# MoonLab-YH/AOD_MEH_HUA

Measured on AMD Instinct MI355X. Metric: images/sec train+HUA-score, RetinaNet-R50 VOC 512^2, higher is better.
Workload: dtype bf16x3

## Files before the change

### aod_meh_hua_amd/_C.py

```python
import ctypes as C
import os

import torch

_HERE = os.path.dirname(os.path.abspath(__file__))
LIB_PATH = os.environ.get('AOD_HIP_LIB') or os.path.join(_HERE, 'lib', 'libaodhip.so')


class AodHipError(RuntimeError):
    pass


if not os.path.exists(LIB_PATH):
    raise ImportError(f'{LIB_PATH} is missing: run `python -m aod_meh_hua_amd.build` (hipcc, gfx950). '
                      'There is no CPU fallback for the MEH/HUA hot path.')
lib = C.CDLL(LIB_PATH)


class ConvSeg(C.Structure):
    _fields_ = [('B', C.c_int32), ('H', C.c_int32), ('W', C.c_int32), ('OH', C.c_int32), ('OW', C.c_int32),
                ('src_row0', C.c_int64), ('dst_row0', C.c_int64)]


class ConvDesc(C.Structure):
    _fields_ = [('C', C.c_int32), ('N', C.c_int32), ('R', C.c_int32), ('S', C.c_int32), ('stride', C.c_int32),
                ('pad', C.c_int32), ('dil', C.c_int32), ('transposed', C.c_int32), ('relu', C.c_int32),
                ('out_f32', C.c_int32), ('nseg', C.c_int32), ('x3', C.c_int32), ('seg', ConvSeg * 8)]


class ConvPlan(C.Structure):
    _fields_ = [(n, C.c_int32) for n in ('kind', 'bm', 'bn', 'nt', 'ops', 'stages', 'x3', 'grouped', 'ksplit', 'taps', 'wide', 'pre', 'lat', 'grid')]


P, I32, I64, F32, U64, SZ = C.c_void_p, C.c_int32, C.c_int64, C.c_float, C.c_uint64, C.c_size_t
_SIGS = {
    'aod_version': (C.c_int, []),
    'aod_conv_x3p_count': (C.c_int64, []),
    'aod_set_pointwise_mode': (C.c_int, [I32]),
    'aod_bottleneck64_fwd': (C.c_int, [P, I32, I32, I32, I32, P, P, P, P, P, P, P, P, P, P, P, P]),
    'aod_bottleneck64x3_fwd': (C.c_int, [P, I32, I32, I32, I32, P, P, P, P, P, P, P, P, P, P, P, P]),
    'aod_bottleneck64x3_ds_fwd': (C.c_int, [P, I32, I32, I32, P, P, P, P, P, P, P, P, P, P, P, P, P, P]),
    'aod_bottleneck64_ds_fwd': (C.c_int, [P, I32, I32, I32, P, P, P, P, P, P, P, P, P, P, P, P, P, P]),
    'aod_halo_conv3x3_x3_applies': (C.c_int, [P]),
    'aod_halo_conv3x3_x3': (C.c_int, [P, P, P, P, P, P]),
    'aod_mfma_clock_probe': (C.c_int, [I32, I32, P, P, P]),
    'aod_bottleneck128x3_bwd': (C.c_int, [P, I32, I32, I32, P, P, P, P, P, P, P, P, P, P, P, P, P]),
    'aod_bottleneck128x3_fwd': (C.c_int, [P, I32, I32, I32, P, P, P, P, P, P, P, P, P, P, P, P, P]),
    'aod_bottleneck128_fwd': (C.c_int, [P, I32, I32, I32, P, P, P, P, P, P, P, P, P, P, P, P, P]),
    'aod_frag_pack': (C.c_int, [P, I32, I32, P]),
    'aod_frag_pack_item_bytes': (C.c_int, []),
    'aod_bottleneck256f_fwd': (C.c_int, [P, I32, I32, I32, P, P, P, P, P, P, P, P, P, P, P, P, P]),
    'aod_bottleneck256f_bwd': (C.c_int, [P, I32, I32, I32, P, P, P, P, P, P, P, P, P, P, P, P, P]),
    'aod_bottleneck_bwd': (C.c_int, [I32, P, I32, I32, I32, P, P, P, P, P, P, P, P, P, P, P, P, P]),
    'aod_bottleneck256_fwd': (C.c_int, [P, I32, I32, I32, P, P, P, P, P, P, P, P, P, P, P, P, P]),
    'aod_conv2d': (C.c_int, [C.POINTER(ConvDesc), P, P, P, P, P, P, P, P, P, P, P]),
    'aod_conv2d_ws_bytes': (SZ, [C.POINTER(ConvDesc)]),
    'aod_conv2d_ws': (C.c_int, [C.POINTER(ConvDesc), P, P, P, P, P, P, P, P, P, P, P, SZ, P]),
    'aod_conv2d_plan': (C.c_int, [C.POINTER(ConvDesc), I32, C.c_uint, C.POINTER(ConvPlan)]),
    'aod_conv2d_grouped': (C.c_int, [C.POINTER(ConvDesc), I32, P, P, P, P, P, P, P]),
    'aod_halo_conv3x3_applies': (C.c_int, [C.POINTER(ConvDesc)]),
    'aod_halo_conv3x3': (C.c_int, [C.POINTER(ConvDesc), P, P, P, P, P, P, P]),
    'aod_conv2d_wgrad': (C.c_int, [C.POINTER(ConvDesc), P, P, P, P, P]),
    'aod_conv2d_wgrad_splits': (C.c_int, [C.POINTER(ConvDesc)]),
    'aod_conv2d_wgrad_slabs': (C.c_int, [C.POINTER(ConvDesc), P, P, P, I32, I64, P, P]),
    'aod_conv2d_wgrad_group_plan': (C.c_int, [P, I32, P]),
    'aod_conv2d_wgrad_grouped': (C.c_int, [P, I32, P, P, P, P, P, P, P]),
    'aod_unpack_wgrad_slabs_grouped': (C.c_int, [I32, P, P, P, P, P, P, P, P, P, P, P, P, P, P, P, P, P]),
    'aod_unpack_wgrad_slabs': (C.c_int, [P, I32, I64, P, I32, I32, I32, I32, I32, I32, P, P, P, P, P, P, P]),
    'aod_conv_row_table_bytes': (SZ, [C.POINTER(ConvDesc)]),
    'aod_conv_row_table': (C.c_int, [C.POINTER(ConvDesc), P, P]),
    'aod_pack_weight_fwd': (C.c_int, [P, P, I32, I32, I32, I32, I32, P]),
    'aod_param_prep': (C.c_int, [P, I32, I32, P]),
    'aod_param_prep_item_bytes': (C.c_int, []),
    'aod_pack_weight_dgrad': (C.c_int, [P, P, I32, I32, I32, I32, I32, P, P]),
    'aod_unpack_wgrad': (C.c_int, [P, P, I32, I32, I32, I32, I32, I32, I32, P, P, P, P, P, P, P]),
    'aod_nchw_f32_to_nhwc_bf16': (C.c_int, [P, P, I32, I32, I32, I32, I32, P]),
    'aod_nchw_f32_to_s2d_bf16': (C.c_int, [P, P, I32, I32, I32, I32, P]),
    'aod_stem_pool_fwd': (C.c_int, [P, P, P, P, P, I32, I32, I32, P]),
    'aod_set_deterministic': (C.c_int, [I32]),
    'aod_get_deterministic': (C.c_int, []),
    'aod_stem_pool_x3_fwd': (C.c_int, [P, P, P, P, P, I32, I32, I32, I32, P]),
    'aod_maxpool3x3s2': (C.c_int, [P, P, I32, I32, I32, I32, P]),
    'aod_upsample2x_add': (C.c_int, [P, P, I32, I32, I32, I32, I32, I32, P]),
    'aod_upsample2x_add_bwd': (C.c_int, [P, P, I32, I32, I32, I32, I32, I32, P]),
# ... 79 lines not shown
```

### aod_meh_hua_amd/csrc/conv.hip

```cpp
#include "common.h"
#include "pointwise.h"
#include "conv_x3p.h"

struct ConvGroup { const bf16_t* x; const bf16_t* w; void* y; const float* pre_shift; const bf16_t* mask; float* colsum; };
struct ConvKParams {
  const bf16_t* x;
  const bf16_t* w;
  void* y;
  const float* pre_scale;
  const float* pre_shift;
  const bf16_t* res;
  const bf16_t* mask;
  const float* post_scale;
  bf16_t* zraw;
  float* colsum;
  int C, N, K, R, S, stride, pad, dil, transposed, relu, out_f32;
  int nseg, M;
  int tiles_m, tiles_n;
  int ksplit;
  float* ws;
  int perm;
  int ngroups;
  ConvGroup grp[4];
  int stagger;
  int x3;
  int tap_inner;
  int bigrows;
  float* cs_ws;
  int up_w, up_hw;
  long long x_bytes, w_bytes;
  int segH[8], segW[8], segOH[8], segOW[8], segB[8];
  long long seg_src0[8], seg_dst0[8];
  int seg_mend[8];
};

#ifdef AOD_TILE_TIMING
__device__ unsigned long long* g_tile_stamps = nullptr;
extern "C" int aod_dbg_set_tile_stamps(void* buf) { return (int)hipMemcpyToSymbol(HIP_SYMBOL(g_tile_stamps), &buf, sizeof(buf)); }
#define TSTAMP(k) do { if (g_tile_stamps && threadIdx.x == 0) g_tile_stamps[(size_t)blockIdx.x * 16 + (k)] = wall_clock64(); } while (0)
#else
#define TSTAMP(k) do {} while (0)
#endif

__device__ __forceinline__ unsigned udiv_small(unsigned n, unsigned d) {
  unsigned q = (unsigned)((float)n * __builtin_amdgcn_rcpf((float)d));
  const int r = (int)(n - q * d);
  q = r < 0 ? q - 1 : ((unsigned)r >= d ? q + 1 : q);
  return q;
}

__device__ __forceinline__ int xcd_swizzle(int bid, int nwg) {
  const int q = nwg >> 3, r = nwg & 7, xcd = bid & 7, j = bid >> 3;
  return (xcd < r ? xcd * (q + 1) : r * (q + 1) + (xcd - r) * q) + j;
}

template <int BM, int BN, int NT, int OPS, bool GROUPED, int ST, bool X3>
__global__ __launch_bounds__(NT) __attribute__((amdgpu_waves_per_eu(BM >= 192 ? 2 : (NT == 512 ? 4 : 1), BM >= 192 ? 2 : (NT == 512 ? 4 : 8)))) void conv_igemm_kernel(const ConvKParams p) {
  static_assert(NT == 256 || NT == 512, "4 or 8 waves");
  static_assert(ST == 2 || (ST == 3 && NT == 256), "LDS stages: 2, or 3 for the 4-wave forms");
  static_assert(!X3 || NT == 256 || (NT == 512 && (BM == 256 || BM == 192 || BM == 128)), "X3: the 4-wave forms, the 8-wave 256 x 256 / 192 x 192 tiles and (A/B) the 8-wave 128 x 128 tile");
  constexpr int BK = 64;
  constexpr int CPR = BK / 8;
  constexpr int RPP = NT / CPR;
  constexpr int A_IT = BM / RPP, B_IT = BN / RPP;
  constexpr int ROWB = BK * 2;
  constexpr int A_BYTES = BM * ROWB, B_BYTES = BN * ROWB, STAGE = A_BYTES + B_BYTES;
  constexpr int WAVES_M = NT / 128;
  constexpr int WM = BM / WAVES_M, WN = BN / 2;
  constexpr int MI = WM / 16, NI = WN / 16;
  constexpr int CP = BN + 4;
  constexpr int EP = (BM * CP * 4 > 144 * 1024) ? 2 : 1;
  constexpr int EBM = BM / EP;
  constexpr bool PREFETCH = EP == 1 && !X3;
  extern __shared__ __attribute__((aligned(16))) char smem[];

  const int t = threadIdx.x;
  TSTAMP(0);
  const int lane = t & 63, wave = t >> 6;
  const int wm = wave >> 1, wn = wave & 1;
  const int nwg = p.tiles_m * p.tiles_n;
  int wg;
  if (!p.perm) wg = xcd_swizzle(blockIdx.x, nwg * (GROUPED ? p.ngroups : p.ksplit));
  else if ((nwg & 31) == 0) {
    const int x = blockIdx.x & 7, j = blockIdx.x >> 3, q = j & 3, k = j >> 2, tq = nwg >> 2;
    wg = q * tq + x * (tq >> 3) + k;
  } else wg = blockIdx.x;
  const int tile = wg % nwg, zz = wg / nwg;
  const int kz = GROUPED ? 0 : zz;
  const int gi = GROUPED ? zz : 0;
#define AOD_GSEL(f, dflt) (GROUPED ? (gi == 0 ? p.grp[0].f : (gi == 1 ? p.grp[1].f : (gi == 2 ? p.grp[2].f : p.grp[3].f))) : (dflt))
  const bf16_t* const g_x = AOD_GSEL(x, p.x);
  const bf16_t* const g_w = AOD_GSEL(w, p.w);
  const float* const g_shift = AOD_GSEL(pre_shift, p.pre_shift);
#define g_y AOD_GSEL(y, p.y)
#define g_mask AOD_GSEL(mask, p.mask)
#define g_colsum AOD_GSEL(colsum, p.colsum)
  const int tile_n = tile % p.tiles_n, tile_m = tile / p.tiles_n;
  const int m0 = tile_m * BM, n0 = tile_n * BN;
#ifdef AOD_TILE_TIMING
  if (m0 < 0) return;
  TSTAMP(8);
#endif

  const int uw = __builtin_amdgcn_readfirstlane(wave);
  const int prow = lane >> 3;
  const int kc = (lane & 7) ^ ((4 * uw + (lane >> 4)) & 7);
  const int C8 = p.C >> 3;
  const auto rsrc_x = __builtin_amdgcn_make_buffer_rsrc((void*)g_x, 0, (int)p.x_bytes, 0x00020000);
  const auto rsrc_w = __builtin_amdgcn_make_buffer_rsrc((void*)g_w, 0, (int)p.w_bytes, 0x00020000);
  constexpr unsigned OOB = 0xfffffff0u;

  unsigned rbase[A_IT];
  int ry0[A_IT], rx0[A_IT], rH[A_IT], rW[A_IT];
  auto seg_of = [&](int m) {
    int sg = 0;
    if (p.nseg > 1) {
#pragma unroll
      for (int q = 0; q < 7; ++q) sg += (m >= p.seg_mend[q]) ? 1 : 0;
    }
    return sg;
  };
  const int m_last = (m0 + BM < p.M ? m0 + BM : p.M) - 1;
  const int sg_first = seg_of(m0);
  const bool one_seg = sg_first == seg_of(m_last);
  struct Geo { unsigned mstart, OW, OH, ohw, B, H, W, src0b, imgb; };
  auto load_geo = [&](int sg) {
    Geo g;
    g.mstart = sg ? (unsigned)p.seg_mend[sg - 1] : 0u;
    g.OW = (unsigned)p.segOW[sg]; g.OH = (unsigned)p.segOH[sg]; g.ohw = g.OH * g.OW; g.B = (unsigned)p.segB[sg];
    g.H = (unsigned)p.segH[sg]; g.W = (unsigned)p.segW[sg];
    g.src0b = (unsigned)((unsigned long long)p.seg_src0[sg] * (unsigned)(p.C * 2));
    g.imgb = g.H * g.W * (unsigned)(p.C * 2);
    return g;
  };
  const Geo gu = load_geo(sg_first);
  auto udiv = [&](unsigned n, unsigned d) { return p.bigrows ? n / d : udiv_small(n, d); };
  auto rowpos = [&](unsigned ml, const Geo& g, unsigned& b, unsigned& oy, unsigned& ox, int& cls) {
    if (!p.perm) {
      b = udiv(ml, g.ohw);
      const unsigned rem = ml - b * g.ohw;
      oy = udiv(rem, g.OW); ox = rem - oy * g.OW; cls = 0;
    } else {
      const unsigned H0 = (g.OH + 1) >> 1, H1 = g.OH >> 1, W0 = (g.OW + 1) >> 1, W1 = g.OW >> 1;
      const unsigned e0 = g.B * H0 * W0, e1 = e0 + g.B * H0 * W1, e2 = e1 + g.B * H1 * W0;
      cls = (ml >= e0 ? 1 : 0) + (ml >= e1 ? 1 : 0) + (ml >= e2 ? 1 : 0);
      const unsigned start = cls == 0 ? 0u : (cls == 1 ? e0 : (cls == 2 ? e1 : e2));
      const unsigned Hc = (cls & 2) ? H1 : H0, Wc = (cls & 1) ? W1 : W0, hw = Hc * Wc;
      const unsigned r = ml - start;
      b = udiv(r, hw);
      const unsigned rem = r - b * hw, yy = udiv(rem, Wc);
      oy = 2 * yy + (unsigned)(cls >> 1); ox = 2 * (rem - yy * Wc) + (unsigned)(cls & 1);
// ... 563 lines not shown
#pragma unroll
        for (int j = 0; j < 8; ++j) zv[j] = (bf16_t)raw[j];
        *reinterpret_cast<bf16x8*>(p.zraw + off) = zv;
      }
    } else {
      for (int j = 0; j < 8 && n + j < p.N; ++j) {
        const long long off = drow * p.N + n + j;
        float u = v[j];
        if (p.pre_scale) u *= p.pre_scale[n + j];
        if (g_shift) u += g_shift[n + j];
        if (p.res) u += (float)p.res[off];
        if (g_mask) u = ((float)g_mask[off] > 0.f) ? u : 0.f;
        if (p.post_scale) u *= p.post_scale[n + j];
        if (p.relu) u = fmaxf(u, 0.f);
        csum[j] += u;
        if (p.out_f32) reinterpret_cast<float*>(g_y)[off] = u;
        else reinterpret_cast<bf16_t*>(g_y)[off] = (bf16_t)u;
        if (p.zraw) p.zraw[off] = (bf16_t)raw[j];
      }
    }
  }
  }
  TSTAMP(5);
#ifdef AOD_TILE_TIMING
  __builtin_amdgcn_s_waitcnt(0);
  asm volatile("s_waitcnt vmcnt(0)" ::: "memory");
  TSTAMP(6);
  if (g_tile_stamps && threadIdx.x == 0)
    g_tile_stamps[(size_t)blockIdx.x * 16 + 7] = ((unsigned long long)__builtin_amdgcn_s_getreg(63508) << 32) | (unsigned)__builtin_amdgcn_s_getreg(63492);
#endif
  if (g_colsum) {
    __syncthreads();
    float* sr = reinterpret_cast<float*>(smem);
#pragma unroll
    for (int j = 0; j < 8; ++j) if (ecok) sr[er * BN + ec * 8 + j] = csum[j];
    __syncthreads();
    if (t < BN && n0 + t < p.N) {
      float s = 0.f;
      for (int r = 0; r < NT / NCHT; ++r) s += sr[r * BN + t];
      if (p.cs_ws) p.cs_ws[((long long)gi * p.tiles_m + tile_m) * p.N + n0 + t] = s;
      else atomicAdd(g_colsum + n0 + t, s);
    }
  }
}

#undef g_y
#undef g_mask
#undef g_colsum
#undef AOD_GSEL

template <int BM, int BN, int NT = 256, int OPS = 2, bool GROUPED = false, int ST = 2, bool X3 = false>
static int launch_conv(const ConvKParams& p, hipStream_t st) {
  ConvKParams q = p;
  q.tiles_m = (p.M + BM - 1) / BM;
  q.tiles_n = (p.N + BN - 1) / BN;
  const size_t stage = (size_t)(BM + BN) * 128 * ST;
  const size_t epi_full = (size_t)BM * (BN + 4) * 4;
  const size_t epi = epi_full > 144 * 1024 ? epi_full / 2 : epi_full;
  const size_t lds = (stage > epi ? stage : epi) + (size_t)BM * 8;
  static unsigned long long attr_done = 0;
  if (aod_first_on_device(&attr_done)) {
    (void)hipFuncSetAttribute(reinterpret_cast<const void*>(&conv_igemm_kernel<BM, BN, NT, OPS, GROUPED, ST, X3>), hipFuncAttributeMaxDynamicSharedMemorySize, (int)lds);
  }
  bool any_cs = q.colsum != nullptr;
  if (GROUPED) for (int g = 0; g < q.ngroups; ++g) any_cs = any_cs || q.grp[g].colsum;
  const int ng = GROUPED ? q.ngroups : 1;
  if (q.ksplit == 1) q.cs_ws = any_cs ? aod_det_scratch((size_t)ng * q.tiles_m * q.N) : nullptr;
  hipLaunchKernelGGL((conv_igemm_kernel<BM, BN, NT, OPS, GROUPED, ST, X3>), dim3(q.tiles_m * q.tiles_n * (q.ngroups > 1 ? q.ngroups : q.ksplit)), dim3(NT), lds, st, q);
  if (q.ksplit == 1 && q.cs_ws) {
    for (int g = 0; g < ng; ++g) {
      float* dst = GROUPED ? q.grp[g].colsum : q.colsum;
      if (dst) { const int rc = aod_colsum_finalize(q.cs_ws + (size_t)g * q.tiles_m * q.N, q.tiles_m, q.N, q.N, dst, nullptr, 0, st); if (rc) return rc; }
    }
  }
  return 0;
}

static int fill_params(const aod_conv_desc_t* d, ConvKParams& p) {
  AOD_CHECK_ARG(d->nseg >= 1 && d->nseg <= 8, "conv: nseg %d out of range", d->nseg);
  AOD_CHECK_ARG(d->C % 8 == 0, "conv: source channels %d must be a multiple of 8", d->C);
  AOD_CHECK_ARG(d->stride >= 1 && d->dil >= 1 && d->R >= 1 && d->S >= 1, "conv: bad geometry");
  AOD_CHECK_ARG(d->x3 == 0 || d->x3 == 1, "conv: aod_conv_desc_t.x3 = %d (0 or 1; descriptors must be zero-initialised -- the field took the place of padding in aod_version() 2)", d->x3);
  p.C = d->C; p.N = d->N; p.R = d->R; p.S = d->S; p.K = d->R * d->S * d->C;
  p.stride = d->stride; p.pad = d->pad; p.dil = d->dil; p.transposed = d->transposed;
  p.relu = d->relu; p.out_f32 = d->out_f32; p.nseg = d->nseg; p.x3 = d->x3 ? 1 : 0;
  if (p.x3) AOD_CHECK_ARG(d->C % 64 == 0, "conv (x3): X-layout source width %d must be a multiple of 64", d->C);
  long long m = 0;
  for (int i = 0; i < d->nseg; ++i) {
    const aod_conv_seg_t& s = d->seg[i];
    if (!d->transposed) {
      const int eh = (s.H + 2 * d->pad - d->dil * (d->R - 1) - 1) / d->stride + 1;
      const int ew = (s.W + 2 * d->pad - d->dil * (d->S - 1) - 1) / d->stride + 1;
      AOD_CHECK_ARG(s.OH >= 1 && s.OW >= 1 && s.OH <= eh && s.OW <= ew, "conv: segment %d output %dx%d exceeds the expected %dx%d", i, s.OH, s.OW, eh, ew);
    } else {
      const int eh = (s.OH + 2 * d->pad - d->dil * (d->R - 1) - 1) / d->stride + 1;
      const int ew = (s.OW + 2 * d->pad - d->dil * (d->S - 1) - 1) / d->stride + 1;
      AOD_CHECK_ARG(eh == s.H && ew == s.W, "dgrad: segment %d dZ %dx%d != expected %dx%d", i, s.H, s.W, eh, ew);
    }
    AOD_CHECK_ARG(s.H < 65536 && s.W < 65536 && s.OH < 65536 && s.OW < 65536, "conv: segment %d image side >= 65536", i);
    p.segB[i] = s.B; p.segH[i] = s.H; p.segW[i] = s.W; p.segOH[i] = s.OH; p.segOW[i] = s.OW;
    p.seg_src0[i] = s.src_row0; p.seg_dst0[i] = s.dst_row0;
    m += (long long)s.B * s.OH * s.OW;
    AOD_CHECK_ARG(m < (1ll << 31), "conv: too many rows");
    p.seg_mend[i] = (int)m;
  }
  for (int i = d->nseg; i < 8; ++i) { p.segB[i] = p.segH[i] = p.segW[i] = p.segOH[i] = p.segOW[i] = 0; p.seg_src0[i] = p.seg_dst0[i] = 0; p.seg_mend[i] = (int)m; }
  p.M = (int)m;
  p.bigrows = 0;
// ... 59 lines not shown
        bf16x8 ov;
#pragma unroll
        for (int j = 0; j < 8; ++j) ov[j] = (bf16_t)v[j];
        *reinterpret_cast<bf16x8*>(reinterpret_cast<bf16_t*>(p.y) + off) = ov;
        if (xout) {
          bf16x8 ol;
#pragma unroll
          for (int j = 0; j < 8; ++j) ol[j] = (bf16_t)(v[j] - (float)ov[j]);
          *reinterpret_cast<bf16x8*>(reinterpret_cast<bf16_t*>(p.y) + off + 32) = ol;
        }
      } else {
        for (int j = 0; j < 8 && n + j < p.N; ++j) {
          if (p.out_f32) reinterpret_cast<float*>(p.y)[off + j] = v[j];
          else reinterpret_cast<bf16_t*>(p.y)[off + j] = (bf16_t)v[j];
        }
      }
      if (p.zraw)
        for (int j = 0; j < 8 && n + j < p.N; ++j) p.zraw[off + j] = (bf16_t)raw[j];
    }
  }
  if (p.colsum) {
#pragma unroll
    for (int j = 0; j < 8; ++j) sr[er][ec * 8 + j] = csum[j];
    __syncthreads();
    const int c = blockIdx.y * 256 + t;
    if (c < p.N) {
      float s2 = 0.f;
#pragma unroll
      for (int r = 0; r < 8; ++r) s2 += sr[r][t];
      if (p.cs_ws) p.cs_ws[(long long)blockIdx.x * p.N + c] = s2;
      else atomicAdd(p.colsum + c, s2);
    }
  }
}

struct ConvKnobs {
  struct Once {
    const char* ksplit_maxhw = getenv("AOD_KSPLIT_MAXHW");
    const char* ksplit_steps = getenv("AOD_KSPLIT_STEPS");
    const char* stagger = getenv("AOD_STAGGER");
    const char* x3_taps_inner = getenv("AOD_X3_TAPS_INNER");
    const char* dgrad_lattice = getenv("AOD_DGRAD_LATTICE");
    const char* dgrad_classes = getenv("AOD_DGRAD_CLASSES");
    const char* tile_want = getenv("AOD_TILE_WANT");
    const char* tile_256 = getenv("AOD_TILE_256");
    const char* x3_128_w8 = getenv("AOD_X3_128_W8");
    const char* x3_128_st3 = getenv("AOD_X3_128_ST3");
    const char* tile_w8 = getenv("AOD_TILE_W8");
    const char* ring3 = getenv("AOD_RING3");
  };
  static const Once& once() { static const Once k{}; return k; }

  enum Call { X3P_OVER_256, X3_TILE_192, X3P_GROUPED, X3P, X3P_PRE, X3P_BN, X3P_DGRAD, X3P_LATTICE, X3P_MIN_STEPS, X3P_PRE_MIN_STEPS, X3P_MIN_TILES,
              X3P_ROT, NCALL };
  const char* val[NCALL];
  unsigned seen = 0;
  const char* call(Call k) {
    static const char* const names[NCALL] = {"AOD_X3P_OVER_256", "AOD_X3_TILE_192", "AOD_X3P_GROUPED", "AOD_X3P", "AOD_X3P_PRE", "AOD_X3P_BN",
                                             "AOD_X3P_DGRAD", "AOD_X3P_LATTICE", "AOD_X3P_MIN_STEPS", "AOD_X3P_PRE_MIN_STEPS", "AOD_X3P_MIN_TILES",
                                             "AOD_X3P_ROT"};
    if (!((seen >> k) & 1u)) { val[k] = getenv(names[k]); seen |= 1u << k; }
    return val[k];
  }
  bool is(Call k, char c) { const char* v = call(k); return v && v[0] == c; }
};
static bool knob_is(const char* v, char c) { return v && v[0] == c; }

static int xp_cus() {
  static int cus[64];
  int dev = 0;
  if (hipGetDevice(&dev) != hipSuccess || dev < 0 || dev > 63) return 256;
  if (!cus[dev]) {
    int n = 0;
    if (hipDeviceGetAttribute(&n, hipDeviceAttributeMultiprocessorCount, dev) != hipSuccess || n <= 0) n = 256;
    cus[dev] = n;
  }
  return cus[dev];
}

static int choose_ksplit(const ConvKParams& p) {
  const ConvKnobs::Once& k1 = ConvKnobs::once();
  const int nk = (p.K + 63) / 64;
  if (nk < 64) return 1;
  const long long maxhw = k1.ksplit_maxhw ? atoll(k1.ksplit_maxhw) : 256;
  long long rows16 = 0;
  for (int i = 0; i < p.nseg; ++i) {
    if (p.segB[i] <= 0) continue;
    if ((long long)p.segOH[i] * p.segOW[i] > maxhw) return 1;
    rows16 += 16ll * p.segOH[i] * p.segOW[i];
  }
  if (k1.ksplit_steps) { const int per = atoi(k1.ksplit_steps); return nk / per > 1 ? nk / per : 1; }
  const long long tiles = ((rows16 + 127) / 128) * ((p.N + 127) / 128);
  long long ks = 512 / (tiles > 0 ? tiles : 1);
  if (ks > nk / 8) ks = nk / 8;
  return ks > 1 ? (int)ks : 1;
}

static int conv_params(const aod_conv_desc_t* desc, const void* src, const void* w_packed, void* dst, const float* pre_scale,
                       const float* pre_shift, const void* res, const void* mask, const float* post_scale, void* zraw, float* colsum,
                       ConvKParams& p) {
  AOD_CHECK_ARG(desc && src && w_packed && dst, "conv: null pointer");
  memset(&p, 0, sizeof(p));
  int rc = fill_params(desc, p);
  if (rc) return rc;
  AOD_CHECK_ARG(!(desc->out_f32 && zraw), "conv: zraw needs a bf16 destination");
  if (desc->x3) {
    AOD_CHECK_ARG(!zraw && !post_scale, "conv (x3): zraw / post_scale are not supported");
    AOD_CHECK_ARG(desc->out_f32 || desc->N % 32 == 0, "conv (x3): a bf16 (X-layout) destination needs N %% 32 == 0, got %d", desc->N);
    AOD_CHECK_ARG(!(desc->out_f32 && (res || mask)), "conv (x3): residual / mask operands need an X-layout destination");
  }
  const ConvKnobs::Once& k1 = ConvKnobs::once();
  p.x = (const bf16_t*)src; p.w = (const bf16_t*)w_packed; p.y = dst;
  p.pre_scale = pre_scale; p.pre_shift = pre_shift; p.res = (const bf16_t*)res; p.mask = (const bf16_t*)mask;
// ... 81 lines not shown
  if (det_colsum) return false;
  if ((long long)p.K * 2 * p.N >= 0x7fffffffll) return false;
  const long long rows = lat == 1 ? (long long)p.segB[0] * (p.segOH[0] / 2) * (p.segOW[0] / 2) : p.M;
  const long long tiles_m = (rows + XP_BM - 1) / XP_BM, reps = (long long)ng * (lat == 1 ? 4 : 1);
  int pre = 0;
  if (taps == 1 && lat == 0 && ngroups <= 1 && p.stride == 1 && (p.res != nullptr) != (p.mask != nullptr) && !kn.is(ConvKnobs::X3P_PRE, '0'))
    pre = p.res ? 1 : 2;
  const int ncu = xp_cus();
  bool wide = false;
  if (!pre && p.N % 256 == 0) {
    const char* fbn = kn.call(ConvKnobs::X3P_BN);
    wide = fbn ? atoi(fbn) == 256 : tiles_m * (p.N / 256) * reps >= (long long)ncu * 3 / 4;
  }
  {
    const char* ms = kn.call(ConvKnobs::X3P_MIN_STEPS);
    const int thr = ms ? atoi(ms) : 24;
    const int steps = lat == 1 ? 9 * (p.C >> 6) / 4 : taps * (p.C >> 6);
    const char* pms = kn.call(ConvKnobs::X3P_PRE_MIN_STEPS);
    if (pms && pre) { if (steps < atoi(pms)) return false; }
    else if (lat != 1 && (steps * (wide ? 2 : 1) < thr || (p.res && steps < thr))) return false;
    if (lat == 1 && steps * (wide ? 2 : 1) < thr / 2) return false;
  }
  long long prev = 0;
  for (int i = 0; i < p.nseg; ++i) {
    const long long r = p.seg_mend[i] - prev;
    prev = p.seg_mend[i];
    if (r >= (1ll << 22)) return false;
    if (i + 1 < p.nseg && r % XP_BM != 0) return false;
    if (p.seg_dst0[i] + r >= (1ll << 31)) return false;
  }
  const char* mint = kn.call(ConvKnobs::X3P_MIN_TILES);
  if (tiles_m * (p.N / 128) * reps < (mint ? atoll(mint) : 192)) return false;
  const long long ntiles = tiles_m * (p.N / (wide ? 256 : 128)) * reps;
  out.kind = AOD_CONV_PLAN_X3P;
  out.taps = lat == 1 ? 4 : taps;
  out.wide = wide; out.pre = pre; out.lat = lat; out.x3 = 1; out.grouped = ngroups ? 1 : 0;
  out.grid = (int)(ntiles < ncu ? ntiles : ncu);
  return true;
}

static int conv_plan(const ConvKParams& p, int ngroups, bool has_workspace, ConvPlan& out) {
  memset(&out, 0, sizeof(out));
  const ConvKnobs::Once& k1 = ConvKnobs::once();
  ConvKnobs kn;
  bool any_mask = p.mask != nullptr, any_cs = p.colsum != nullptr;
  for (int g = 0; g < ngroups; ++g) { any_mask = any_mask || p.grp[g].mask; any_cs = any_cs || p.grp[g].colsum; }
  auto igemm = [&](int bm, int bn, int nt, int ops, int stages) {
    out.kind = AOD_CONV_PLAN_IGEMM; out.bm = bm; out.bn = bn; out.nt = nt; out.ops = ops; out.stages = stages; out.x3 = p.x3; out.grouped = ngroups ? 1 : 0;
    return 0;
  };
  auto w8 = [&](int bm, int bn) { return igemm(bm, bn, 512, any_mask ? 1 : 0, 2); };
  auto ntiles = [&](int bm, int bn) { return (long long)((p.M + bm - 1) / bm) * ((p.N + bn - 1) / bn); };
  const long long t256 = ntiles(256, 256);
  const bool fits256 = t256 >= 240 && t256 * 100 >= ((t256 + 255) / 256) * 256 * 92;
  const bool shape256 = !p.res && !p.out_f32 && p.N % 256 == 0 && p.K >= (p.x3 ? 2048 : 1024);
  const long long want = k1.tile_want ? atoll(k1.tile_want) : 512;

  if (ngroups) {
    if (p.x3 && p.R == p.S && !p.bigrows && kn.is(ConvKnobs::X3P_GROUPED, '1') && plan_x3p(p, ngroups, any_cs && aod_get_deterministic(), kn, out)) return 0;
    if (p.x3) return w8(256, 256);
    auto fill = [&](int bm, int bn, int slots) {
      const long long t = ntiles(bm, bn) * ngroups;
      return (double)t / (double)(((t + slots - 1) / slots) * slots);
    };
    const bool ok256 = !knob_is(k1.tile_256, '0') && p.N % 256 == 0 && p.K >= 1024;
    if (ok256 && fill(256, 256, 256) * 1.12 >= fill(128, 128, 512)) return w8(256, 256);
    AOD_CHECK_ARG(p.N >= 128, "conv_grouped: N >= 128 required");
    return w8(128, 128);
  }

  if (!p.x3 && !p.up_w && p.R == 1 && p.S == 1 && p.stride == 1 && p.pad == 0 && p.nseg == 1 && !p.out_f32 && !p.zraw && !p.post_scale) {
    PwArgs a;
    pw_args(p, a);
    if (aod_pw_wants(a)) { out.kind = AOD_CONV_PLAN_PW_STREAM; return 0; }
  }
  const int ks = (has_workspace && !p.perm && !p.up_w) ? choose_ksplit(p) : 1;
  if (ks > 1) {
    igemm(128, p.N > 64 ? 128 : 64, 256, 2, 2);
    out.kind = AOD_CONV_PLAN_SPLIT_K; out.ksplit = ks;
    return 0;
  }
  if (p.x3) {
    if (!p.out_f32 && !p.zraw && !p.post_scale && !p.bigrows && p.R == p.S && (!(shape256 && fits256) || kn.is(ConvKnobs::X3P_OVER_256, '1')) &&
        plan_x3p(p, 0, any_cs && aod_get_deterministic(), kn, out)) return 0;
    if (!knob_is(k1.tile_256, '0') && shape256 && fits256) return w8(256, 256);
    if (p.N > 128 && p.N <= 192 && !p.res && !p.mask && !p.zraw && p.K >= 2048 && ntiles(192, 192) >= 240 && !kn.is(ConvKnobs::X3_TILE_192, '0'))
      return igemm(192, 192, 512, 0, 2);
    if (knob_is(k1.x3_128_w8, '1') && !p.res && !p.out_f32 && p.N % 128 == 0 && ntiles(128, 128) >= 256) return w8(128, 128);
  } else {
    if (!knob_is(k1.tile_256, '0') && shape256 && ((knob_is(k1.tile_256, '1') && t256 >= 128) || fits256)) return w8(256, 256);
    if (!knob_is(k1.tile_w8, '0') && !p.res && p.N >= 128 && p.K >= 1024 && ntiles(128, 128) >= want) return w8(128, 128);
  }
  const int pad128 = (p.N + 127) / 128 * 128, pad64 = (p.N + 63) / 64 * 64;
  const bool ragged = p.N > 128 && (pad128 - pad64) * 5 >= pad128;
  const int st64 = (p.x3 || (!knob_is(k1.ring3, '0') && p.K >= 256)) ? 3 : 2;
  if (ragged && ntiles(128, 64) >= want) return igemm(128, 64, 256, 2, 2);
  if (p.N > 64 && p.x3 && knob_is(k1.x3_128_st3, '1') && ntiles(128, 128) >= 256) return igemm(128, 128, 256, 2, 3);
  if (p.N > 64 && ntiles(128, 128) >= want) return igemm(128, 128, 256, 2, 2);
  if (p.N > 64 && ntiles(64, 128) >= want) return igemm(64, 128, 256, 2, st64);
  if (p.N <= 64 && ntiles(128, 64) >= want) return igemm(128, 64, 256, 2, 2);
  if (p.N > 64 && ntiles(128, 64) >= want && p.N % 128 != 0) return igemm(128, 64, 256, 2, 2);
  return igemm(64, 64, 256, 2, st64);
}

static void x3p_args(const ConvKParams& p, const ConvPlan& plan, X3PArgs& a) {
  memset(&a, 0, sizeof(a));
  a.x = p.x; a.w = p.w; a.y = reinterpret_cast<bf16_t*>(p.y); a.pre_scale = p.pre_scale; a.pre_shift = p.pre_shift; a.res = p.res; a.mask = p.mask;
  a.colsum = p.colsum; a.C = p.C; a.N = p.N; a.K = p.K; a.taps = p.R * p.S; a.S = p.S; a.stride = p.stride; a.pad = p.pad; a.dil = p.dil;
  a.transposed = p.transposed; a.relu = p.relu; a.nseg = p.nseg; a.M = p.M; a.x_bytes = p.x_bytes; a.w_bytes = p.w_bytes;
  a.tapin = (p.tap_inner && a.taps > 1 && p.C >= 256) ? 1 : 0;
  for (int i = 0; i < 8; ++i) {
    a.segH[i] = p.segH[i]; a.segW[i] = p.segW[i]; a.segOH[i] = p.segOH[i]; a.segOW[i] = p.segOW[i]; a.segB[i] = p.segB[i];
    a.seg_src0[i] = p.seg_src0[i]; a.seg_dst0[i] = p.seg_dst0[i]; a.seg_mend[i] = p.seg_mend[i];
  }
  a.ngroups = p.ngroups > 1 ? p.ngroups : 1;
  a.grp[0].x = a.x; a.grp[0].w = a.w; a.grp[0].y = a.y; a.grp[0].shift = a.pre_shift; a.grp[0].mask = a.mask; a.grp[0].colsum = a.colsum;
  for (int g = 0; g < p.ngroups; ++g) {
    a.grp[g].x = p.grp[g].x; a.grp[g].w = p.grp[g].w; a.grp[g].y = reinterpret_cast<bf16_t*>(p.grp[g].y); a.grp[g].shift = p.grp[g].pre_shift;
    a.grp[g].mask = p.grp[g].mask; a.grp[g].colsum = p.grp[g].colsum;
  }
  a.lat = plan.lat; a.up_w = p.up_w; a.up_hw = p.up_hw;
  const long long rows = a.lat == 1 ? (long long)a.segB[0] * (a.segOH[0] / 2) * (a.segOW[0] / 2) : a.M;
  a.tiles_m = (int)((rows + XP_BM - 1) / XP_BM);
  a.tiles_n = a.N / (plan.wide ? 256 : 128);
}

#define CONV_IGEMM_INSTANCES(X)                                                                                                       \
  X(256, 256, 512, 0, false, 2, false) X(256, 256, 512, 1, false, 2, false) X(128, 128, 512, 0, false, 2, false) X(128, 128, 512, 1, false, 2, false) \
  X(128, 128, 256, 2, false, 2, false) X(128, 64, 256, 2, false, 2, false) X(64, 128, 256, 2, false, 2, false) X(64, 128, 256, 2, false, 3, false)   \
  X(64, 64, 256, 2, false, 2, false) X(64, 64, 256, 2, false, 3, false)                                                               \
  X(256, 256, 512, 0, true, 2, false) X(256, 256, 512, 1, true, 2, false) X(128, 128, 512, 0, true, 2, false) X(128, 128, 512, 1, true, 2, false)    \
  X(256, 256, 512, 0, false, 2, true) X(256, 256, 512, 1, false, 2, true) X(192, 192, 512, 0, false, 2, true)                          \
  X(128, 128, 512, 0, false, 2, true) X(128, 128, 512, 1, false, 2, true) X(128, 128, 256, 2, false, 2, true) X(128, 128, 256, 2, false, 3, true)    \
  X(128, 64, 256, 2, false, 2, true) X(64, 128, 256, 2, false, 3, true) X(64, 64, 256, 2, false, 3, true)                              \
  X(256, 256, 512, 0, true, 2, true) X(256, 256, 512, 1, true, 2, true)

static int launch_igemm(const ConvPlan& pl, const ConvKParams& p, hipStream_t st) {
#define X(BM, BN, NT, OPS, GROUPED, ST, X3)                                                                                           \
  if (pl.bm == BM && pl.bn == BN && pl.nt == NT && pl.ops == OPS && (pl.grouped != 0) == GROUPED && pl.stages == ST && (pl.x3 != 0) == X3) \
    return launch_conv<BM, BN, NT, OPS, GROUPED, ST, X3>(p, st);
  CONV_IGEMM_INSTANCES(X)
#undef X
  AOD_CHECK_ARG(false, "conv: no kernel instance for the plan %d x %d, %d threads, ops %d, %d stages, x3 %d, grouped %d", pl.bm, pl.bn, pl.nt, pl.ops,
                pl.stages, pl.x3, pl.grouped);
  return -1;
}

static int conv_launch(const ConvPlan& pl, ConvKParams& p, void* workspace, size_t workspace_bytes, hipStream_t st) {
  switch (pl.kind) {
    case AOD_CONV_PLAN_PW_STREAM: {
      PwArgs a;
      pw_args(p, a);
      return aod_pw_gemm(a, st);
    }
    case AOD_CONV_PLAN_X3P: {
      X3PArgs a;
      x3p_args(p, pl, a);
      ConvKnobs kn;
      const char* r = kn.call(ConvKnobs::X3P_ROT);
      a.rot = r ? atoi(r) : 0;
      return aod_conv_x3p_launch(a, pl, st);
    }
    case AOD_CONV_PLAN_SPLIT_K: {
      const size_t need = (size_t)pl.ksplit * p.M * p.N * 4;
      AOD_CHECK_ARG(workspace && workspace_bytes >= need, "conv: split-K workspace of %zu bytes, need %zu (aod_conv2d_ws_bytes)", workspace_bytes, need);
      p.ksplit = pl.ksplit; p.ws = (float*)workspace;
      int rc = launch_igemm(pl, p, st);
      if (rc) return rc;
      AOD_LAUNCH_CHECK();
      p.cs_ws = p.colsum ? aod_det_scratch((size_t)((p.M + 7) / 8) * p.N) : nullptr;
      hipLaunchKernelGGL(conv_splitk_finalize_kernel, dim3((p.M + 7) / 8, (p.N + 255) / 256), dim3(256), 0, st, p);
      AOD_LAUNCH_CHECK();
      if (p.cs_ws) return aod_colsum_finalize(p.cs_ws, (p.M + 7) / 8, p.N, p.N, p.colsum, nullptr, 0, st);
      return 0;
    }
    case AOD_CONV_PLAN_IGEMM: {
      int rc = launch_igemm(pl, p, st);
      if (rc) return rc;
      AOD_LAUNCH_CHECK();
      return 0;
    }
  }
  AOD_CHECK_ARG(false, "conv: plan of unknown kind %d", pl.kind);
  return -1;
}

extern "C" int aod_conv2d_ws(const aod_conv_desc_t* desc, const void* src, const void* w_packed, void* dst,
                             const float* pre_scale, const float* pre_shift, const void* res, const void* mask,
                             const float* post_scale, void* zraw, float* colsum, void* workspace, size_t workspace_bytes,
                             aod_stream_t stream) {
  ConvKParams p;
  ConvPlan pl;
  int rc = conv_params(desc, src, w_packed, dst, pre_scale, pre_shift, res, mask, post_scale, zraw, colsum, p);
  if (rc) return rc;
  if (p.M == 0) return 0;
  rc = conv_plan(p, 0, workspace != nullptr, pl);
  if (rc) return rc;
  return conv_launch(pl, p, workspace, workspace_bytes, (hipStream_t)stream);
}

extern "C" int aod_conv2d_grouped(const aod_conv_desc_t* desc, int ngroups, const void* const* src, const void* const* w_packed,
                                  void* const* dst, const float* const* pre_shift, const void* const* mask, float* const* colsum,
                                  aod_stream_t stream) {
  ConvKParams p;
  ConvPlan pl;
  int rc = conv_params_grouped(desc, ngroups, src, w_packed, dst, pre_shift, mask, colsum, p);
  if (rc) return rc;
  if (p.M == 0) return 0;
  rc = conv_plan(p, ngroups, false, pl);
  if (rc) return rc;
  return conv_launch(pl, p, nullptr, 0, (hipStream_t)stream);
}

extern "C" int aod_conv2d(const aod_conv_desc_t* desc, const void* src, const void* w_packed, void* dst,
                          const float* pre_scale, const float* pre_shift, const void* res, const void* mask,
                          const float* post_scale, void* zraw, float* colsum, aod_stream_t stream) {
  return aod_conv2d_ws(desc, src, w_packed, dst, pre_scale, pre_shift, res, mask, post_scale, zraw, colsum, nullptr, 0, stream);
}

extern "C" int aod_conv2d_plan(const aod_conv_desc_t* desc, int ngroups, unsigned operand_flags, aod_conv_plan_t* out) {
  AOD_CHECK_ARG(desc && out && ngroups >= 0 && ngroups <= 4, "conv_plan: null pointer or ngroups outside 0..4");
  static char operand[16];
  char* const dst = operand + 8;
  auto has = [&](unsigned f) { return (operand_flags & f) ? (void*)operand : nullptr; };
  void* const res = (operand_flags & AOD_CONV_RES_IS_DST) ? (void*)dst : has(AOD_CONV_HAS_RES);
  ConvKParams p;
  int rc;
  if (ngroups) {
    const void* in[4] = {operand, operand, operand, operand};
// ... 1054 lines not shown
```

### include/aod_hip.h

```cpp
#ifndef AOD_HIP_H
#define AOD_HIP_H
#include <stddef.h>
#include <stdint.h>

#ifdef __cplusplus
extern "C" {
#endif

typedef void* aod_stream_t;

const char* aod_last_error(void);
int aod_version(void);

typedef struct {
  int32_t B, H, W;
  int32_t OH, OW;
  int64_t src_row0;
  int64_t dst_row0;
} aod_conv_seg_t;

typedef struct {
  int32_t C, N;
  int32_t R, S;
  int32_t stride, pad, dil;
  int32_t transposed;
  int32_t relu;
  int32_t out_f32;
  int32_t nseg;
  int32_t x3;
  aod_conv_seg_t seg[8];
} aod_conv_desc_t;

int aod_conv2d(const aod_conv_desc_t* desc, const void* src, const void* w_packed, void* dst,
               const float* pre_scale, const float* pre_shift, const void* res, const void* mask,
               const float* post_scale, void* zraw, float* colsum, aod_stream_t stream);

size_t aod_conv2d_ws_bytes(const aod_conv_desc_t* desc);
int aod_conv2d_ws(const aod_conv_desc_t* desc, const void* src, const void* w_packed, void* dst,
                  const float* pre_scale, const float* pre_shift, const void* res, const void* mask,
                  const float* post_scale, void* zraw, float* colsum, void* workspace, size_t workspace_bytes,
                  aod_stream_t stream);

enum { AOD_CONV_PLAN_PW_STREAM = 1,
       AOD_CONV_PLAN_SPLIT_K = 2,
       AOD_CONV_PLAN_X3P = 3,
       AOD_CONV_PLAN_IGEMM = 4 };
enum { AOD_CONV_HAS_PRE_SCALE = 1, AOD_CONV_HAS_PRE_SHIFT = 2, AOD_CONV_HAS_RES = 4, AOD_CONV_RES_IS_DST = 8, AOD_CONV_HAS_MASK = 16,
       AOD_CONV_HAS_POST_SCALE = 32, AOD_CONV_HAS_ZRAW = 64, AOD_CONV_HAS_COLSUM = 128, AOD_CONV_HAS_WORKSPACE = 256 };
typedef struct {
  int32_t kind;
  int32_t bm, bn, nt, ops, stages, x3, grouped;
  int32_t ksplit;
  int32_t taps, wide, pre, lat, grid;
} aod_conv_plan_t;
int aod_conv2d_plan(const aod_conv_desc_t* desc, int ngroups, unsigned operand_flags, aod_conv_plan_t* out);

int64_t aod_conv_x3p_count(void);

int aod_set_pointwise_mode(int mode);

int aod_set_deterministic(int on);
int aod_get_deterministic(void);

int aod_bottleneck64_fwd(const void* x, int Cin, int B, int H, int W, const void* w1, const float* s1, const float* b1, const void* w2,
                         const float* s2, const float* b2, const void* w3, const float* s3, const float* b3, const void* res, void* y,
                         aod_stream_t stream);
int aod_bottleneck64_ds_fwd(const void* x, int B, int H, int W, const void* w1, const float* s1, const float* b1, const void* w2,
                            const float* s2, const float* b2, const void* w3, const float* s3, const float* b3, const void* wd,
                            const float* sd, const float* bd, void* y, aod_stream_t stream);
int aod_bottleneck128_fwd(const void* x, int B, int H, int W, const void* w1, const float* s1, const float* b1, const void* w2,
                          const float* s2, const float* b2, const void* w3, const float* s3, const float* b3, void* y, void* t1, void* t2,
                          aod_stream_t stream);
int aod_bottleneck256_fwd(const void* x, int B, int H, int W, const void* w1, const float* s1, const float* b1, const void* w2,
                          const float* s2, const float* b2, const void* w3, const float* s3, const float* b3, void* y, void* t1, void* t2,
                          aod_stream_t stream);
int aod_bottleneck_bwd(int planes, const void* g, int B, int H, int W, const void* wd3, const void* wd2, const void* wd1, const void* act_t2,
                       const void* act_t1, const void* act_x, void* gx, void* gt2, void* gt1, float* colsum_t2, float* colsum_t1,
                       float* colsum_x, aod_stream_t stream);

int aod_frag_pack_item_bytes(void);
int aod_frag_pack(const void* items_dev, int nitems, int total_blocks, aod_stream_t stream);
int aod_bottleneck256f_fwd(const void* x, int B, int H, int W, const void* w1f, const float* s1, const float* b1, const void* w2f,
                           const float* s2, const float* b2, const void* w3f, const float* s3, const float* b3, void* y, void* t1, void* t2,
                           aod_stream_t stream);
int aod_bottleneck256f_bwd(const void* g, int B, int H, int W, const void* wd3f, const void* wd2f, const void* wd1f, const void* act_t2,
                           const void* act_t1, const void* act_x, void* gx, void* gt2, void* gt1, float* colsum_t2, float* colsum_t1,
                           float* colsum_x, aod_stream_t stream);

int aod_conv2d_grouped(const aod_conv_desc_t* desc, int ngroups, const void* const* src, const void* const* w_packed, void* const* dst,
                       const float* const* pre_shift, const void* const* mask, float* const* colsum, aod_stream_t stream);

int aod_conv2d_wgrad(const aod_conv_desc_t* desc, const void* x, const void* dz, float* dw_f32,
                     const void* row_table, aod_stream_t stream);
int aod_conv2d_wgrad_splits(const aod_conv_desc_t* desc);
int aod_conv2d_wgrad_slabs(const aod_conv_desc_t* desc, const void* x, const void* dz, float* slabs, int nslabs, int64_t slab_stride,
                           const void* row_table, aod_stream_t stream);
int aod_conv2d_wgrad_group_plan(const aod_conv_desc_t* const* descs, int n, int32_t* splits_out);
int aod_conv2d_wgrad_grouped(const aod_conv_desc_t* const* descs, int n, const void* const* x, const void* const* dz, float* const* slabs,
                             const int32_t* nslabs, const int64_t* slab_stride, const void* const* row_table, aod_stream_t stream);
size_t aod_conv_row_table_bytes(const aod_conv_desc_t* desc);
int aod_conv_row_table(const aod_conv_desc_t* desc, void* table, aod_stream_t stream);

int aod_pack_weight_fwd(const float* w_oihw, void* w_packed, int O, int I, int R, int S, int Ipad, aod_stream_t stream);
int aod_pack_weight_dgrad(const float* w_oihw, void* w_packed, int O, int I, int R, int S, int Opad, const float* scale,
                          aod_stream_t stream);
int aod_unpack_wgrad(float* dw_orsi, float* grad_oihw, int O, int I, int R, int S, int Ipad, int accumulate, int clear_src,
// ... 182 lines not shown
```

Before: 629.6.

## Split 256x256 conv launches into main body plus narrower tail wave

When a 256x256-tile implicit-GEMM conv leaves a small partial last wave over the CU slots, the planner now splits the launch: the bulk of row tiles run with 256x256 tiles and the trailing row tiles run as a second launch with 256x128 tiles. This adds row-tile offset/count fields to the kernel params and plan, new kernel instantiations, and heuristics comparing against x3p and 128x128 plans. It aims to cut wave-quantization idle time on the last wave, at the cost of an extra launch and more planning complexity.

After: 633.2, median of 6. About the same (+0.6%).

```diff
diff --git a/aod_meh_hua_amd/_C.py b/aod_meh_hua_amd/_C.py
--- a/aod_meh_hua_amd/_C.py
+++ b/aod_meh_hua_amd/_C.py
@@ -29,7 +29,8 @@
 
 
 class ConvPlan(C.Structure):
-    _fields_ = [(n, C.c_int32) for n in ('kind', 'bm', 'bn', 'nt', 'ops', 'stages', 'x3', 'grouped', 'ksplit', 'taps', 'wide', 'pre', 'lat', 'grid')]
+    _fields_ = [(n, C.c_int32) for n in ('kind', 'bm', 'bn', 'nt', 'ops', 'stages', 'x3', 'grouped', 'ksplit', 'taps', 'wide', 'pre', 'lat', 'grid',
+                                             'tail_bn', 'tail_tiles')]
 
 
 P, I32, I64, F32, U64, SZ = C.c_void_p, C.c_int32, C.c_int64, C.c_float, C.c_uint64, C.c_size_t
diff --git a/aod_meh_hua_amd/csrc/conv.hip b/aod_meh_hua_amd/csrc/conv.hip
--- a/aod_meh_hua_amd/csrc/conv.hip
+++ b/aod_meh_hua_amd/csrc/conv.hip
@@ -17,6 +17,7 @@
   int C, N, K, R, S, stride, pad, dil, transposed, relu, out_f32;
   int nseg, M;
   int tiles_m, tiles_n;
+  int tile_m0, tile_cnt;
   int ksplit;
   float* ws;
   int perm;
@@ -96,7 +97,7 @@
 #define g_mask AOD_GSEL(mask, p.mask)
 #define g_colsum AOD_GSEL(colsum, p.colsum)
   const int tile_n = tile % p.tiles_n, tile_m = tile / p.tiles_n;
-  const int m0 = tile_m * BM, n0 = tile_n * BN;
+  const int m0 = (tile_m + p.tile_m0) * BM, n0 = tile_n * BN;
 #ifdef AOD_TILE_TIMING
   if (m0 < 0) return;
   TSTAMP(8);
@@ -766,8 +767,10 @@
 template <int BM, int BN, int NT = 256, int OPS = 2, bool GROUPED = false, int ST = 2, bool X3 = false>
 static int launch_conv(const ConvKParams& p, hipStream_t st) {
   ConvKParams q = p;
-  q.tiles_m = (p.M + BM - 1) / BM;
+  q.tiles_m = p.tile_cnt ? p.tile_cnt : (p.M + BM - 1) / BM - p.tile_m0;
   q.tiles_n = (p.N + BN - 1) / BN;
+  AOD_CHECK_ARG(q.tile_m0 >= 0 && q.tiles_m > 0 && (long long)(q.tile_m0 + q.tiles_m - 1) * BM < p.M, "conv: row tiles %d + %d outside the %d rows", q.tile_m0, q.tiles_m, p.M);
+  AOD_CHECK_ARG((!q.tile_m0 && !q.tile_cnt) || (!GROUPED && q.ksplit == 1 && !q.perm), "conv: a partial row-tile range in a grouped / split-K / class-major launch");
   const size_t stage = (size_t)(BM + BN) * 128 * ST;
   const size_t epi_full = (size_t)BM * (BN + 4) * 4;
   const size_t epi = epi_full > 144 * 1024 ? epi_full / 2 : epi_full;
@@ -933,13 +936,13 @@
   static const Once& once() { static const Once k{}; return k; }
 
   enum Call { X3P_OVER_256, X3_TILE_192, X3P_GROUPED, X3P, X3P_PRE, X3P_BN, X3P_DGRAD, X3P_LATTICE, X3P_MIN_STEPS, X3P_PRE_MIN_STEPS, X3P_MIN_TILES,
-              X3P_ROT, NCALL };
+              X3P_ROT, CONV_TAIL, CONV_SLOTS, NCALL };
   const char* val[NCALL];
   unsigned seen = 0;
   const char* call(Call k) {
     static const char* const names[NCALL] = {"AOD_X3P_OVER_256", "AOD_X3_TILE_192", "AOD_X3P_GROUPED", "AOD_X3P", "AOD_X3P_PRE", "AOD_X3P_BN",
                                              "AOD_X3P_DGRAD", "AOD_X3P_LATTICE", "AOD_X3P_MIN_STEPS", "AOD_X3P_PRE_MIN_STEPS", "AOD_X3P_MIN_TILES",
-                                             "AOD_X3P_ROT"};
+                                             "AOD_X3P_ROT", "AOD_CONV_TAIL", "AOD_CONV_SLOTS"};
     if (!((seen >> k) & 1u)) { val[k] = getenv(names[k]); seen |= 1u << k; }
     return val[k];
   }
@@ -1127,8 +1130,21 @@
   auto w8 = [&](int bm, int bn) { return igemm(bm, bn, 512, any_mask ? 1 : 0, 2); };
   auto ntiles = [&](int bm, int bn) { return (long long)((p.M + bm - 1) / bm) * ((p.N + bn - 1) / bn); };
   const long long t256 = ntiles(256, 256);
-  const bool fits256 = t256 >= 240 && t256 * 100 >= ((t256 + 255) / 256) * 256 * 92;
   const bool shape256 = !p.res && !p.out_f32 && p.N % 256 == 0 && p.K >= (p.x3 ? 2048 : 1024);
+  const bool shape192 = p.x3 && p.N > 128 && p.N <= 192 && !p.res && !p.mask && !p.zraw && p.K >= 2048;
+  long long slots = 256;
+  if (shape256 || shape192) { const char* s = kn.call(ConvKnobs::CONV_SLOTS); if (s && atoi(s) > 0) slots = atoi(s); }
+  auto fills = [&](long long t) { return t * 256 >= 240 * slots && t * 100 >= ((t + slots - 1) / slots) * slots * 92; };
+  const bool fits256 = fills(t256);
+  auto tail256 = [&]() -> int {
+    if (ngroups || !shape256 || fits256 || p.perm || p.up_w || knob_is(k1.tile_256, '0') || aod_get_deterministic()) return 0;
+    const long long tn = p.N / 256, rem = t256 % slots;
+    if (t256 <= slots || rem == 0 || rem * 2 >= slots || rem % tn != 0) return 0;
+    if (kn.is(ConvKnobs::CONV_TAIL, '0')) return 0;
+    return (int)(rem / tn);
+  };
+  auto w8_tail = [&](int tail_rows) { w8(256, 256); out.tail_bn = 128; out.tail_tiles = tail_rows; return 0; };
+  auto tail_q = [&]() { return 4 * (t256 / slots) + ((p.x3 && !kn.is(ConvKnobs::CONV_TAIL, '1')) ? 4 : 2); };
   const long long want = k1.tile_want ? atoll(k1.tile_want) : 512;
 
   if (ngroups) {
@@ -1157,13 +1173,23 @@
   }
   if (p.x3) {
     if (!p.out_f32 && !p.zraw && !p.post_scale && !p.bigrows && p.R == p.S && (!(shape256 && fits256) || kn.is(ConvKnobs::X3P_OVER_256, '1')) &&
-        plan_x3p(p, 0, any_cs && aod_get_deterministic(), kn, out)) return 0;
+        plan_x3p(p, 0, any_cs && aod_get_deterministic(), kn, out)) {
+      const int tr = kn.is(ConvKnobs::X3P_OVER_256, '1') ? 0 : tail256();
+      const long long xt = (long long)((p.M + XP_BM - 1) / XP_BM) * (p.N / (out.wide ? 256 : 128)), ncu = xp_cus();
+      if (!tr || tail_q() > (xt + ncu - 1) / ncu * (out.wide ? 2 : 1)) return 0;
+      memset(&out, 0, sizeof(out));
+      return w8_tail(tr);
+    }
     if (!knob_is(k1.tile_256, '0') && shape256 && fits256) return w8(256, 256);
-    if (p.N > 128 && p.N <= 192 && !p.res && !p.mask && !p.zraw && p.K >= 2048 && ntiles(192, 192) >= 240 && !kn.is(ConvKnobs::X3_TILE_192, '0'))
+    if (const int tr = tail256()) return w8_tail(tr);
+    if (shape192 && ntiles(192, 192) * 256 >= 240 * slots && !kn.is(ConvKnobs::X3_TILE_192, '0'))
       return igemm(192, 192, 512, 0, 2);
     if (knob_is(k1.x3_128_w8, '1') && !p.res && !p.out_f32 && p.N % 128 == 0 && ntiles(128, 128) >= 256) return w8(128, 128);
   } else {
     if (!knob_is(k1.tile_256, '0') && shape256 && ((knob_is(k1.tile_256, '1') && t256 >= 128) || fits256)) return w8(256, 256);
+    if (const int tr = tail256()) {
+      if (tail_q() <= (ntiles(128, 128) + 2 * slots - 1) / (2 * slots) * 2) return w8_tail(tr);
+    }
     if (!knob_is(k1.tile_w8, '0') && !p.res && p.N >= 128 && p.K >= 1024 && ntiles(128, 128) >= want) return w8(128, 128);
   }
   const int pad128 = (p.N + 127) / 128 * 128, pad64 = (p.N + 63) / 64 * 64;
@@ -1208,7 +1234,8 @@
   X(256, 256, 512, 0, false, 2, true) X(256, 256, 512, 1, false, 2, true) X(192, 192, 512, 0, false, 2, true)                          \
   X(128, 128, 512, 0, false, 2, true) X(128, 128, 512, 1, false, 2, true) X(128, 128, 256, 2, false, 2, true) X(128, 128, 256, 2, false, 3, true)    \
   X(128, 64, 256, 2, false, 2, true) X(64, 128, 256, 2, false, 3, true) X(64, 64, 256, 2, false, 3, true)                              \
-  X(256, 256, 512, 0, true, 2, true) X(256, 256, 512, 1, true, 2, true)
+  X(256, 256, 512, 0, true, 2, true) X(256, 256, 512, 1, true, 2, true)                                                                \
+  X(256, 128, 512, 0, false, 2, false) X(256, 128, 512, 1, false, 2, false) X(256, 128, 512, 0, false, 2, true) X(256, 128, 512, 1, false, 2, true)
 
 static int launch_igemm(const ConvPlan& pl, const ConvKParams& p, hipStream_t st) {
 #define X(BM, BN, NT, OPS, GROUPED, ST, X3)                                                                                           \
@@ -1250,6 +1277,22 @@
       return 0;
     }
     case AOD_CONV_PLAN_IGEMM: {
+      if (pl.tail_tiles > 0) {
+        const int all = (p.M + pl.bm - 1) / pl.bm;
+        AOD_CHECK_ARG(pl.tail_tiles < all && pl.tail_bn > 0, "conv: tail of %d row tiles in a launch of %d", pl.tail_tiles, all);
+        p.tile_m0 = 0; p.tile_cnt = all - pl.tail_tiles;
+        int rc = launch_igemm(pl, p, st);
+        if (rc) return rc;
+        AOD_LAUNCH_CHECK();
+        ConvPlan tp = pl;
+        tp.bn = pl.tail_bn;
+        p.tile_m0 = all - pl.tail_tiles; p.tile_cnt = pl.tail_tiles;
+        rc = launch_igemm(tp, p, st);
+        p.tile_m0 = p.tile_cnt = 0;
+        if (rc) return rc;
+        AOD_LAUNCH_CHECK();
+        return 0;
+      }
       int rc = launch_igemm(pl, p, st);
       if (rc) return rc;
       AOD_LAUNCH_CHECK();
diff --git a/include/aod_hip.h b/include/aod_hip.h
--- a/include/aod_hip.h
+++ b/include/aod_hip.h
@@ -52,6 +52,7 @@
   int32_t bm, bn, nt, ops, stages, x3, grouped;
   int32_t ksplit;
   int32_t taps, wide, pre, lat, grid;
+  int32_t tail_bn, tail_tiles;
 } aod_conv_plan_t;
 int aod_conv2d_plan(const aod_conv_desc_t* desc, int ngroups, unsigned operand_flags, aod_conv_plan_t* out);
 
```
